# wangys16/FreeSplat

Measured on AMD Instinct MI355X. Metric: rendered views/sec @ 968x1296, 1.0M Gaussians, higher is better.
Workload: dtype f32

## Files before the change

### freesplat_amd/csrc/fs_common.h

```cpp
#pragma once
#include <hip/hip_runtime.h>
#include <stdint.h>

#include "../../include/freesplat_amd.h"

#define FS_API extern "C" __attribute__((visibility("default")))

namespace fs {

constexpr int kTile = FS_TILE;
constexpr int kTilePix = kTile * kTile;
constexpr int kWave = 64;

void set_last_error(const char* what, hipError_t e);

#define FS_CHECK_LAUNCH(what)                                   \
    do {                                                        \
        hipError_t e__ = hipGetLastError();                     \
        if (e__ != hipSuccess) {                                \
            fs::set_last_error(what, e__);                      \
            return FS_ERR_LAUNCH;                               \
        }                                                       \
    } while (0)

enum Stage {
    kStPreprocess = 0, kStTileScan, kStRender, kStRenderBwd, kStPreprocessBwd,
    kStCostVolume, kStPtf, kStEncoderTail, kNumStages
};
struct ScopedStage {
    ScopedStage(Stage s, hipStream_t st, int units = 1);
    ~ScopedStage();
    int slot_;
    hipStream_t st_;
};

__host__ __device__ inline size_t align_up(size_t x, size_t a) { return (x + a - 1) / a * a; }

constexpr float kExpC1 = 0.9999997019767761f, kExpC2 = 0.4999915063381195f, kExpC3 = 0.1666763573884964f, kExpC4 = 0.04189793020486832f, kExpC5 = 0.008290314115583897f;
__device__ __forceinline__ float fs_exp(float x)
{
    if (x < -80.0f) return 0.0f;
    const float t = fmaf(x, 1.44269504088896341f, 12582912.0f);
    const float n = t - 12582912.0f;
    const float r = fmaf(n, -0.693147182464599609375f, x);
    float p = fmaf(r, kExpC5, kExpC4);
    p = fmaf(r, p, kExpC3);
    p = fmaf(r, p, kExpC2);
    p = fmaf(r, p, kExpC1);
    p = fmaf(r, p, 1.0f);
    return ldexpf(p, (int)n);
}

#ifdef FS_PHASE_TRACE
constexpr int kPtKernels = 4, kPtBlocks = 4096, kPtSlots = 10;
static __device__ unsigned long long g_phase_trace[kPtKernels * kPtBlocks * kPtSlots];
#define FS_PT(kern, k)                                                                                  \
    do {                                                                                                \
        if (threadIdx.x == 0 && blockIdx.x < fs::kPtBlocks)                                             \
            fs::g_phase_trace[((kern) * fs::kPtBlocks + blockIdx.x) * fs::kPtSlots + (k)] = wall_clock64(); \
    } while (0)
#else
#define FS_PT(kern, k) do {} while (0)
#endif

__device__ __forceinline__ void rev2pi(float x, float& rev, float& res)
{
    constexpr float kInv2PiHi = 0.15915494f, kInv2PiLo = 6.4206382e-9f;
    rev = x * kInv2PiHi;
    res = fmaf(x, kInv2PiLo, fmaf(x, kInv2PiHi, -rev));
}
__device__ __forceinline__ void pos_enc2(float a, float b, float* __restrict__ out)
{
    float ra, ea, rb, eb;
    rev2pi(a, ra, ea);
    rev2pi(b, rb, eb);
#pragma unroll
    for (int k = 0; k < 6; ++k) {
        const float f = (float)(1 << k);
        const float ta = ra * f, tb = rb * f;
        const float pa = (ta - rintf(ta)) + ea * f, pb = (tb - rintf(tb)) + eb * f;
        out[2 * k] = __builtin_amdgcn_sinf(pa); out[2 * k + 1] = __builtin_amdgcn_cosf(pa);
        out[12 + 2 * k] = __builtin_amdgcn_sinf(pb); out[12 + 2 * k + 1] = __builtin_amdgcn_cosf(pb);
    }
}

int launch_ptf_gru(int n_max, const int32_t* counts, const float* cat, const float* tables, float* fused, hipStream_t st);
int launch_ptf_gru_gather(int n_max, const int32_t* counts, const long long* fuse_idx, const long long* fuse_pix,
                          const float* G, const float* R, const float* O, const float* g_i, const float* rho_i,
                          const float* om_i, const float* tables, float* fused, bool out_after_keep, hipStream_t st,
                          float* save_side = nullptr, float* save_act = nullptr, float* save_cat = nullptr);

__device__ __forceinline__ void wave_lds_sync()
{
    __builtin_amdgcn_fence(__ATOMIC_RELEASE, "wavefront");
    __builtin_amdgcn_wave_barrier();
    __builtin_amdgcn_fence(__ATOMIC_ACQUIRE, "wavefront");
}

typedef float f32x2 __attribute__((ext_vector_type(2)));
typedef int i32x2 __attribute__((ext_vector_type(2)));
__device__ __forceinline__ f32x2 fma2(f32x2 a, f32x2 b, f32x2 c) { return __builtin_elementwise_fma(a, b, c); }
__device__ __forceinline__ f32x2 splat2(float v) { return (f32x2){v, v}; }

__device__ __forceinline__ f32x2 fs_exp2_nonpos(f32x2 x)
{
    const f32x2 magic = splat2(12582912.0f);
    const f32x2 t = fma2(x, splat2(1.44269504088896341f), magic);
    const f32x2 n = t - magic;
    const f32x2 r = fma2(n, splat2(-0.693147182464599609375f), x);
    f32x2 q = fma2(r, splat2(kExpC5), splat2(kExpC4));
    q = fma2(r, q, splat2(kExpC3));
    q = fma2(r, q, splat2(kExpC2));
    q = fma2(r, q, splat2(kExpC1));
    q = fma2(r, q, splat2(1.0f));
    const i32x2 e = __builtin_bit_cast(i32x2, q) + (__builtin_bit_cast(i32x2, t) << 23);
    return __builtin_bit_cast(f32x2, e);
}

__device__ __forceinline__ f32x2 fs_exp2_of_neg(f32x2 q)
{
    const f32x2 magic = splat2(12582912.0f);
    const f32x2 t = fma2(q, splat2(-1.44269504088896341f), magic);
    const f32x2 n = t - magic;
    const f32x2 r = fma2(n, splat2(-0.693147182464599609375f), -q);
    f32x2 p = fma2(r, splat2(kExpC5), splat2(kExpC4));
    p = fma2(r, p, splat2(kExpC3));
    p = fma2(r, p, splat2(kExpC2));
    p = fma2(r, p, splat2(kExpC1));
    p = fma2(r, p, splat2(1.0f));
    const i32x2 e = __builtin_bit_cast(i32x2, p) + (__builtin_bit_cast(i32x2, t) << 23);
    return __builtin_bit_cast(f32x2, e);
}
template <bool FAST>
__device__ __forceinline__ f32x2 blend_exp_of_neg(f32x2 q)
{
    if constexpr (FAST) {
        const f32x2 t = q * splat2(-1.44269504088896341f);
// ... 223 lines not shown
```

### freesplat_amd/csrc/raster_fwd.hip

```cpp
#include <stdlib.h>

#include <type_traits>

#include "fs_common.h"

namespace fs {

template <int M>
__device__ __forceinline__ uint32_t lane_xor(uint32_t v)
{
    if constexpr (M == 1) return (uint32_t)__builtin_amdgcn_mov_dpp((int)v, 0xB1, 0xF, 0xF, true);
    else if constexpr (M == 2) return (uint32_t)__builtin_amdgcn_mov_dpp((int)v, 0x4E, 0xF, 0xF, true);
    else if constexpr (M == 3) return (uint32_t)__builtin_amdgcn_mov_dpp((int)v, 0x1B, 0xF, 0xF, true);
    else if constexpr (M < 32) return (uint32_t)__builtin_amdgcn_ds_swizzle((int)v, (M << 10) | 0x1F);
    else return (uint32_t)__shfl_xor((int)v, M, 64);
}
template <int M>
__device__ __forceinline__ unsigned long long lane_xor64(unsigned long long v)
{
    const uint32_t lo = lane_xor<M>((uint32_t)v), hi = lane_xor<M>((uint32_t)(v >> 32));
    return ((unsigned long long)hi << 32) | lo;
}

template <int DEG>
__device__ __forceinline__ void eval_sh(const float* __restrict__ sh, float3 dir, float* rgb,
                                        uint8_t& clampbits, int cs, int ks)
{
    float b[16];
    sh_basis<DEG>(dir.x, dir.y, dir.z, b);
    constexpr int NB = (DEG + 1) * (DEG + 1);
    clampbits = 0;
#pragma unroll
    for (int c = 0; c < 3; ++c) {
        const float* s = sh + c * cs;
        float acc = b[0] * s[0];
#pragma unroll
        for (int k = 1; k < NB; ++k) acc = acc + b[k] * s[k * ks];
        acc = acc + 0.5f;
        if (acc < 0.0f) clampbits |= (uint8_t)(1u << c);
        rgb[c] = fmaxf(acc, 0.0f);
    }
}

__device__ __forceinline__ void stage_rows(float* lds, const float* __restrict__ src, size_t base,
                                           int cnt, int per)
{
    const float* s = src + base * per;
    const int total = cnt * per;
    if ((((uintptr_t)s) & 15) == 0) {
        const int nv = total >> 2;
        int k = threadIdx.x;
        for (; k + 768 < nv; k += 1024) {
            const float4 v0 = ((const float4*)s)[k], v1 = ((const float4*)s)[k + 256];
            const float4 v2 = ((const float4*)s)[k + 512], v3 = ((const float4*)s)[k + 768];
            ((float4*)lds)[k] = v0; ((float4*)lds)[k + 256] = v1;
            ((float4*)lds)[k + 512] = v2; ((float4*)lds)[k + 768] = v3;
        }
        for (; k < nv; k += 256) ((float4*)lds)[k] = ((const float4*)s)[k];
        for (int k = (nv << 2) + threadIdx.x; k < total; k += blockDim.x) lds[k] = s[k];
    } else {
        for (int k = threadIdx.x; k < total; k += blockDim.x) lds[k] = s[k];
    }
}



struct QuadForm {
    float a, b, c;
    float Q;
    float D;
    float vplus;
    float Vmax;
    float inv2a;
};
__device__ __forceinline__ QuadForm quad_form(const float4 r0, const float4 r1)
{
    QuadForm f;
    f.a = -r0.z; f.c = -r0.w; f.b = -r1.x;
    f.Q = -(r1.z - 1e-3f * (1.0f + fabsf(r1.z)));
    f.D = 4.0f * f.a * f.c - f.b * f.b;
    const float invD = __builtin_amdgcn_rcpf(f.D);
    const float U = __builtin_amdgcn_sqrtf(fmaxf(4.0f * f.c * f.Q * invD, 0.0f));
    f.vplus = -f.b * __builtin_amdgcn_rcpf(2.0f * f.c) * U;
    f.Vmax = __builtin_amdgcn_sqrtf(fmaxf(4.0f * f.a * f.Q * invD, 0.0f));
    f.inv2a = __builtin_amdgcn_rcpf(2.0f * f.a);
    return f;
}
struct Band { float uL, uR; };
constexpr float kEps = 2e-5f;
__device__ __forceinline__ Band band_interval(const QuadForm& f, float vlo, float vhi)
{
    Band o;
    if (f.Q < 0.0f || vlo > f.Vmax + kEps || vhi < -f.Vmax - kEps) { o.uL = 3.0e38f; o.uR = -3.0e38f; return o; }
    const float vr = fminf(vhi, fmaxf(vlo, f.vplus)), vl = fminf(vhi, fmaxf(vlo, -f.vplus));
    const float sr = __builtin_amdgcn_sqrtf(fmaxf(4.0f * f.a * f.Q - f.D * vr * vr, 0.0f));
    const float sl = __builtin_amdgcn_sqrtf(fmaxf(4.0f * f.a * f.Q - f.D * vl * vl, 0.0f));
    o.uR = (-f.b * vr + sr) * f.inv2a;
    o.uL = (-f.b * vl - sl) * f.inv2a;
    const float w = kEps * (1.0f + fabsf(o.uR) + fabsf(o.uL));
    o.uR += w; o.uL -= w;
    return o;
}
struct RowBands { Band top, bot; };
__device__ __forceinline__ RowBands row_bands(const QuadForm& f, const float4 r0, int ty)
{
    const float v0 = (float)(ty * kTile) - r0.y;
    RowBands r;
    r.top = band_interval(f, v0, v0 + 7.0f);
    r.bot = band_interval(f, v0 + 8.0f, v0 + 15.0f);
    return r;
}
__device__ __forceinline__ uint32_t quad_mask_row(const RowBands& rb, const float4 r0, int tx)
{
    const float u0 = (float)(tx * kTile) - r0.x, u1 = u0 + 8.0f;
    uint32_t m = 0;
    if (!(u0 > rb.top.uR) && !(u0 + 7.0f < rb.top.uL)) m |= 1u;
    if (!(u1 > rb.top.uR) && !(u1 + 7.0f < rb.top.uL)) m |= 2u;
    if (!(u0 > rb.bot.uR) && !(u0 + 7.0f < rb.bot.uL)) m |= 4u;
    if (!(u1 > rb.bot.uR) && !(u1 + 7.0f < rb.bot.uL)) m |= 8u;
    return m;
}

__device__ __forceinline__ uint32_t band_cells(const Band& b, float px, int cell0, int ncell)
{
    const uint32_t full = ncell >= 32 ? 0xFFFFFFFFu : ((1u << ncell) - 1u);
    if (b.uL > b.uR) return 0u;
    if (!(b.uL <= b.uR)) return full;
    const float lo_f = ceilf((b.uL + px - 7.0f) * 0.125f - 1e-3f), hi_f = floorf((b.uR + px) * 0.125f + 1e-3f);
    const int lo = max((int)lo_f, cell0) - cell0, hi = min((int)hi_f, cell0 + ncell - 1) - cell0;
    if (lo > hi) return 0u;
    return ((2u << hi) - (1u << lo)) & full;
}
__device__ __forceinline__ unsigned long long pack_quad_masks(const QuadForm& f, const float4 r0, ushort4 rc)
{
    unsigned long long m = 0;
    const int rw = rc.z - rc.x, cell0 = 2 * rc.x, ncell = 2 * rw;
    int k = 0;
    for (int y = rc.y; y < rc.w; ++y) {
        const RowBands rb = row_bands(f, r0, y);
        const uint32_t top = band_cells(rb.top, r0.x, cell0, ncell), bot = band_cells(rb.bot, r0.x, cell0, ncell);
        for (int x = 0; x < rw; ++x, ++k) {
            const uint32_t nib = ((top >> (2 * x)) & 3u) | (((bot >> (2 * x)) & 3u) << 2);
            m |= (unsigned long long)nib << (4 * k);
        }
    }
    return m;
}

__device__ __forceinline__ uint32_t spread2(uint32_t x)
{
    x = (x | (x << 4)) & 0x0F0Fu;
    return (x | (x << 2)) & 0x3333u;
}
__device__ __forceinline__ unsigned long long pack_quad_masks4(const QuadForm& f, const float4 r0, ushort4 rc, bool cull, uint32_t& nz)
{
    unsigned long long m = 0;
    const int rw = rc.z - rc.x, rh = rc.w - rc.y, cell0 = 2 * rc.x, ncell = 2 * rw;
    const uint32_t rowfull = (1u << rw) - 1u;
    nz = 0u;
#pragma unroll
    for (int r = 0; r < 4; ++r) {
        if (r < rh) {
            const RowBands rb = row_bands(f, r0, rc.y + r);
            const uint32_t top = band_cells(rb.top, r0.x, cell0, ncell), bot = band_cells(rb.bot, r0.x, cell0, ncell);
            m |= (unsigned long long)(spread2(top) | (spread2(bot) << 2)) << (16 * r);
            uint32_t any = top | bot;
            any = (any | (any >> 1)) & 0x55u;
            any = (any | (any >> 1)) & 0x33u;
            any = (any | (any >> 2)) & 0x0Fu;
            nz |= (cull ? any : rowfull) << (4 * r);
        }
    }
    return m;
}

__device__ __forceinline__ void stage_rows_half(float* lds, const _Float16* __restrict__ src, size_t base, int cnt,
                                                int per)
{
    const _Float16* s = src + base * per;
    const int total = cnt * per;
    typedef _Float16 half8 __attribute__((ext_vector_type(8)));
    int done = 0;
    if ((((uintptr_t)s) & 15) == 0) {
        const int nv = total >> 3;
        auto put = [&](int k, const half8 v) {
            ((float4*)lds)[2 * k] = make_float4((float)v[0], (float)v[1], (float)v[2], (float)v[3]);
            ((float4*)lds)[2 * k + 1] = make_float4((float)v[4], (float)v[5], (float)v[6], (float)v[7]);
        };
        int k = threadIdx.x;
        for (; k + 256 < nv; k += 512) {
            const half8 v0 = ((const half8*)s)[k], v1 = ((const half8*)s)[k + 256];
            put(k, v0); put(k + 256, v1);
        }
        for (; k < nv; k += 256) put(k, ((const half8*)s)[k]);
        done = nv << 3;
    }
    for (int k = done + threadIdx.x; k < total; k += blockDim.x) lds[k] = (float)s[k];
}

struct Projected {
    float4 r0, r1, r2;
    ushort4 rect;
    uint8_t cb;
    int rad;
};
__device__ __forceinline__ Projected project_gaussian(
    const fs_raster_dims& d, bool live, float3 p_in, const float (&c_in)[6], float op, size_t i,
    const float* __restrict__ colors, const float* sh , int sh_cs, int sh_ks,
    const float* __restrict__ view, const float* __restrict__ proj, const float* __restrict__ campos,
    float tanfovx, float tanfovy, bool rescale, float wscale)
{
    Projected o;
    o.r0 = make_float4(0, 0, 0, 0); o.r1 = o.r0; o.r2 = o.r0;
    o.rect = make_ushort4(0, 0, 0, 0);
    o.cb = 0;
    o.rad = 0;
    float3 p = p_in;
    if (rescale) { p.x = p.x * wscale; p.y = p.y * wscale; p.z = p.z * wscale; }
    const float3 pv = xform43(view, p);
    if (live && pv.z > 0.2f) {
        const float4 ph = xform44(proj, p);
        const float pw = 1.0f / (ph.w + 0.0000001f);
        const float ndcx = ph.x * pw, ndcy = ph.y * pw;
        const float fx = (float)d.W / (2.0f * tanfovx), fy = (float)d.H / (2.0f * tanfovy);
        float c3[6];
#pragma unroll
        for (int k = 0; k < 6; ++k) c3[k] = c_in[k];
        if (rescale) {
            const float s2 = wscale * wscale;
#pragma unroll
            for (int k = 0; k < 6; ++k) c3[k] = c3[k] * s2;
        }
        const Cov2D cv = project_cov(view, p, c3, fx, fy, tanfovx, tanfovy);
        const float det = cv.a * cv.c - cv.b * cv.b;
        if (det != 0.0f) {
            const float det_inv = 1.0f / det;
            const float cA = cv.c * det_inv, cB = -cv.b * det_inv, cC = cv.a * det_inv;
            const float mid = 0.5f * (cv.a + cv.c);
            const float sq = sqrtf(fmaxf(0.1f, mid * mid - det));
            const float l1 = mid + sq, l2 = mid - sq;
            const float my_radius = ceilf(3.0f * sqrtf(fmaxf(l1, l2)));
            const float px = ((ndcx + 1.0f) * (float)d.W - 1.0f) * 0.5f;
            const float py = ((ndcy + 1.0f) * (float)d.H - 1.0f) * 0.5f;
            const int r = (int)my_radius;
            const int gx = (d.W + kTile - 1) / kTile, gy = (d.H + kTile - 1) / kTile;
            const int x0 = min(gx, max(0, (int)((px - (float)r) / (float)kTile)));
            const int y0 = min(gy, max(0, (int)((py - (float)r) / (float)kTile)));
            const int x1 = min(gx, max(0, (int)((px + (float)r + (float)(kTile - 1)) / (float)kTile)));
            const int y1 = min(gy, max(0, (int)((py + (float)r + (float)(kTile - 1)) / (float)kTile)));
            if ((x1 - x0) * (y1 - y0) > 0) {
                float rgb[3];
                if (colors) {
                    rgb[0] = colors[3 * i];
                    rgb[1] = colors[3 * i + 1];
                    rgb[2] = colors[3 * i + 2];
                } else {
                    float3 dir = make_float3(p.x - campos[0], p.y - campos[1], p.z - campos[2]);
                    const float len = sqrtf(dir.x * dir.x + dir.y * dir.y + dir.z * dir.z);
                    dir.x = dir.x / len; dir.y = dir.y / len; dir.z = dir.z / len;
                    switch (d.sh_degree) {
                        case 0: eval_sh<0>(sh, dir, rgb, o.cb, sh_cs, sh_ks); break;
                        case 1: eval_sh<1>(sh, dir, rgb, o.cb, sh_cs, sh_ks); break;
                        case 2: eval_sh<2>(sh, dir, rgb, o.cb, sh_cs, sh_ks); break;
                        default: eval_sh<3>(sh, dir, rgb, o.cb, sh_cs, sh_ks); break;
                    }
                }
                float thr;
                if (op > 0.0f) {
                    const float l = -logf(255.0f * op);
                    thr = l - (0.001f + 1e-5f * fabsf(l));
                } else {
                    thr = 1.0f;
                }
                o.r0 = make_float4(px, py, -0.5f * cA, -0.5f * cC);
                o.r1 = make_float4(-cB, op, thr, pv.z);
                o.r2 = make_float4(rgb[0], rgb[1], rgb[2], 0.0f);
                o.rect = make_ushort4((unsigned short)x0, (unsigned short)y0, (unsigned short)x1,
                                      (unsigned short)y1);
                o.rad = r;
            }
        }
    }
    return o;
}

template <bool SR>
__device__ __forceinline__ void load_mean_cov(const fs_raster_dims& d, const float* __restrict__ means3D,
                                              const float* __restrict__ cov3D, size_t i, float3& p_in, float (&c_in)[6])
{
    p_in = make_float3(means3D[3 * i], means3D[3 * i + 1], means3D[3 * i + 2]);
    if constexpr (SR) {
        float row[7];
#pragma unroll
        for (int k = 0; k < 7; ++k) row[k] = cov3D[7 * i + k];
        cov_from_scale_rot(row, c_in);
    } else if (d.flags & FS_RASTER_COV_FULL) {
        const float* cr = cov3D + 9 * i;
        c_in[0] = cr[0]; c_in[1] = cr[1]; c_in[2] = cr[2]; c_in[3] = cr[4]; c_in[4] = cr[5]; c_in[5] = cr[8];
    } else {
#pragma unroll
        for (int k = 0; k < 6; ++k) c_in[k] = cov3D[6 * i + k];
    }
}

constexpr int kWaveBins = 512;

__device__ __forceinline__ void bin_wave(const fs_raster_dims& d, int lane, uint32_t* s_cnt, uint32_t i, const Projected& pr,
                                         uint32_t* __restrict__ tile_counts, unsigned long long* __restrict__ keys,
                                         uint32_t tile_cap)
{
    const float4 r0 = pr.r0, r1 = pr.r1;
    const ushort4 rect = pr.rect;
    const bool valid = pr.rad > 0;
    const bool cull = (d.flags & FS_RASTER_TILE_CULL) != 0;
    const int gx = (d.W + kTile - 1) / kTile;
    const QuadForm qf = quad_form(r0, r1);
    const int rw = rect.z - rect.x, rh = rect.w - rect.y;
    const int area = rw * rh;
    const bool small = area <= 16;
    const bool all4 = __builtin_amdgcn_ballot_w64(valid && (rw > 4 || rh > 4)) == 0ull;
    unsigned long long qm = 0;
    uint32_t nz = 0u;
    if (all4) { if (valid) qm = pack_quad_masks4(qf, r0, rect, cull, nz); }
    else if (valid && small) qm = pack_quad_masks(qf, r0, rect);
    const unsigned long long key_hi = ((unsigned long long)__float_as_uint(r1.w) << 32) | (i << 4);
    int x0 = valid ? (int)rect.x : 0x7fff, y0 = valid ? (int)rect.y : 0x7fff;
    int x1 = valid ? (int)rect.z : 0, y1 = valid ? (int)rect.w : 0;
#define FS_BOX_STEP(M)                                                                                           \
    {                                                                                                            \
        const int lo = (int)lane_xor<M>((uint32_t)((x0 << 16) | y0)), hi = (int)lane_xor<M>((uint32_t)((x1 << 16) | y1)); \
        x0 = min(x0, lo >> 16); y0 = min(y0, lo & 0xffff);                                                       \
        x1 = max(x1, hi >> 16); y1 = max(y1, hi & 0xffff);                                                       \
    }
    FS_BOX_STEP(32) FS_BOX_STEP(16) FS_BOX_STEP(8) FS_BOX_STEP(4) FS_BOX_STEP(2) FS_BOX_STEP(1)
#undef FS_BOX_STEP
    const int bx0 = __builtin_amdgcn_readfirstlane(x0), by0 = __builtin_amdgcn_readfirstlane(y0);
    const int bw = max(0, __builtin_amdgcn_readfirstlane(x1) - bx0), bh = max(0, __builtin_amdgcn_readfirstlane(y1) - by0);
    const int nb = bw * bh;
    if (nb == 0) return;
    if (nb <= kWaveBins && all4) {
        for (int k = lane; k < nb; k += 64) s_cnt[k] = 0u;
        wave_lds_sync();
        const int cbase = (rect.y - by0) * bw + (rect.x - bx0);
        for (uint32_t z = nz; z != 0u; z &= z - 1u) {
            const int k = __builtin_ctz(z);
            atomicAdd(&s_cnt[cbase + (k >> 2) * bw + (k & 3)], 1u);
        }
        wave_lds_sync();
        for (int k0 = 0; k0 < nb; k0 += 64) {
            const int k = k0 + lane;
            if (k < nb) {
                const uint32_t c = s_cnt[k];
                const int ky = k / bw, kx = k - ky * bw;
                s_cnt[k] = c ? atomicAdd(&tile_counts[(by0 + ky) * gx + bx0 + kx], c) : 0u;
            }
        }
        wave_lds_sync();
        const uint32_t tbase = (uint32_t)(rect.y * gx + rect.x);
        for (uint32_t z = nz; z != 0u; z &= z - 1u) {
            const int k = __builtin_ctz(z);
            const uint32_t m = (uint32_t)(qm >> (4 * k)) & 15u;
            const uint32_t slot = atomicAdd(&s_cnt[cbase + (k >> 2) * bw + (k & 3)], 1u);
            if (slot < tile_cap) keys[(tbase + (uint32_t)((k >> 2) * gx + (k & 3))) * tile_cap + slot] = key_hi | m;
        }
        wave_lds_sync();
    } else if (nb <= kWaveBins) {
        for (int k = lane; k < nb; k += 64) s_cnt[k] = 0u;
        wave_lds_sync();
        if (valid) {
            int k = 0;
            for (int y = rect.y; y < rect.w; ++y) {
                RowBands rb = {};
                if (!small) rb = row_bands(qf, r0, y);
                for (int x = rect.x; x < rect.z; ++x, ++k) {
                    const uint32_t m = small ? (uint32_t)(qm >> (4 * k)) & 15u : quad_mask_row(rb, r0, x);
                    if (!cull || m) atomicAdd(&s_cnt[(y - by0) * bw + (x - bx0)], 1u);
                }
            }
        }
        wave_lds_sync();
        for (int k0 = 0; k0 < nb; k0 += 64) {
            const int k = k0 + lane;
            if (k < nb) {
                const uint32_t c = s_cnt[k];
                const int ky = k / bw, kx = k - ky * bw;
                s_cnt[k] = c ? atomicAdd(&tile_counts[(by0 + ky) * gx + bx0 + kx], c) : 0u;
            }
        }
        wave_lds_sync();
        if (valid) {
            int k = 0;
            for (int y = rect.y; y < rect.w; ++y) {
                RowBands rb = {};
                if (!small) rb = row_bands(qf, r0, y);
                for (int x = rect.x; x < rect.z; ++x, ++k) {
                    const uint32_t m = small ? (uint32_t)(qm >> (4 * k)) & 15u : quad_mask_row(rb, r0, x);
                    if (!cull || m) {
                        const uint32_t slot = atomicAdd(&s_cnt[(y - by0) * bw + (x - bx0)], 1u);
                        if (slot < tile_cap) keys[(uint32_t)(y * gx + x) * tile_cap + slot] = key_hi | m;
                    }
                }
            }
        }
        wave_lds_sync();
    } else if (all4) {
        const uint32_t tbase = (uint32_t)(rect.y * gx + rect.x);
        for (uint32_t z = nz; z != 0u; z &= z - 1u) {
            const int k = __builtin_ctz(z);
            const uint32_t m = (uint32_t)(qm >> (4 * k)) & 15u;
            const uint32_t tile = tbase + (uint32_t)((k >> 2) * gx + (k & 3));
            const uint32_t slot = atomicAdd(&tile_counts[tile], 1u);
            if (slot < tile_cap) keys[tile * tile_cap + slot] = key_hi | m;
        }
    } else if (valid) {
        int k = 0;
        for (int y = rect.y; y < rect.w; ++y) {
            RowBands rb = {};
            if (!small) rb = row_bands(qf, r0, y);
            for (int x = rect.x; x < rect.z; ++x, ++k) {
                const uint32_t m = small ? (uint32_t)(qm >> (4 * k)) & 15u : quad_mask_row(rb, r0, x);
                if (!cull || m) {
                    const uint32_t slot = atomicAdd(&tile_counts[y * gx + x], 1u);
                    if (slot < tile_cap) keys[(uint32_t)(y * gx + x) * tile_cap + slot] = key_hi | m;
                }
            }
        }
    }
}

__global__ __launch_bounds__(256) void zero_counts_kernel(char* base, size_t stride, int T)
{
    const int k = blockIdx.x * 256 + threadIdx.x;
    if (k < T) ((uint32_t*)(base + stride * blockIdx.y))[k] = 0u;
}

struct ViewBuffers {
    char* geom; size_t geom_stride;
    char* scratch; size_t scratch_stride;
    int32_t* radii;
};

#ifndef FS_PRE_WAVES
#define FS_PRE_WAVES 6
#endif
#define FS_PRE_OCC __attribute__((amdgpu_waves_per_eu(FS_PRE_WAVES, FS_PRE_WAVES)))
template <int CH, bool SR>
__global__ __launch_bounds__(256) FS_PRE_OCC void preprocess_views_kernel(
    fs_raster_dims d, int v, const float* __restrict__ means3D, const float* __restrict__ cov3D,
    const float* __restrict__ shs, const float* __restrict__ colors, const float* __restrict__ opacities,
    const float* __restrict__ view, const float* __restrict__ proj, const float* __restrict__ campos,
    const float* __restrict__ tanfov_dev, const float* __restrict__ scale_dev, ViewBuffers vb, uint32_t tile_cap)
{
    extern __shared__ __attribute__((aligned(16))) float lds[];
    constexpr int kPerBlock = 64 * CH;
    const int base = blockIdx.x * kPerBlock;
    const int cnt = min(kPerBlock, d.N - base);
    const int per_sh = shs ? d.M * 3 : 0;
    const bool sh_cm = (d.flags & FS_RASTER_SH_CHANNEL_MAJOR) != 0;
    const int sh_cs = sh_cm ? d.M : 1, sh_ks = sh_cm ? 1 : 3;
    float* const l_sh = lds;
    if (shs) {
        if (d.flags & FS_RASTER_SH_FP16) stage_rows_half(l_sh, (const _Float16*)shs, base, cnt, per_sh);
        else stage_rows(l_sh, shs, base, cnt, per_sh);
    }
    const int t = threadIdx.x, lane = t & 63, wave = t >> 6;
    const int chunk = wave % CH;
    uint32_t* const s_cnt_base = (uint32_t*)(lds + (size_t)kPerBlock * per_sh);
    uint32_t* const s_cnt = s_cnt_base + wave * kWaveBins;
    const int li = chunk * 64 + lane;
    const bool live = li < cnt;
    const uint32_t i = (uint32_t)(base + li);
    float* const l_g = (float*)(s_cnt_base + 4 * kWaveBins) + li;
    {
        float3 p_in = make_float3(0.0f, 0.0f, 0.0f);
        float c_in[6] = {0, 0, 0, 0, 0, 0};
        float op = 0.0f;
        if (live) {
            load_mean_cov<SR>(d, means3D, cov3D, i, p_in, c_in);
            op = opacities[i];
        }
        if (wave < CH) {
            l_g[0 * kPerBlock] = p_in.x; l_g[1 * kPerBlock] = p_in.y; l_g[2 * kPerBlock] = p_in.z;
#pragma unroll
            for (int k = 0; k < 6; ++k) l_g[(3 + k) * kPerBlock] = c_in[k];
            l_g[9 * kPerBlock] = op;
        }
    }
    __syncthreads();
    const int T = num_tiles(d.H, d.W);
    const size_t keys_off = align_up((size_t)T * 4, 256);
#pragma nounroll
    for (int j0 = wave / CH; j0 < v; j0 += 4 / CH) {
        const int j = __builtin_amdgcn_readfirstlane(j0);
        int li_ = li, lane_ = lane;
        asm volatile("" : "+v"(li_), "+v"(lane_));
        const float* const lg = (const float*)(s_cnt_base + 4 * kWaveBins) + li_;
        const float3 p_in = make_float3(lg[0 * kPerBlock], lg[1 * kPerBlock], lg[2 * kPerBlock]);
        float c_in[6];
#pragma unroll
        for (int k = 0; k < 6; ++k) c_in[k] = lg[(3 + k) * kPerBlock];
        const float op = lg[9 * kPerBlock];
        const float tanfovx = tanfov_dev ? tanfov_dev[2 * j] : d.tanfovx;
        const float tanfovy = tanfov_dev ? tanfov_dev[2 * j + 1] : d.tanfovy;
        const float wscale = scale_dev ? scale_dev[j] : 1.0f;
        const Projected pr = project_gaussian(d, live, p_in, c_in, op, i, colors, l_sh + (size_t)li_ * per_sh, sh_cs, sh_ks,
                                              view + 16 * j, proj + 16 * j, campos + 3 * j, tanfovx, tanfovy,
                                              scale_dev != nullptr, wscale);
        if (live) {
            const GeomView g = geom_view(vb.geom + vb.geom_stride * j, d.N);
            g.rec[3 * (size_t)i + 0] = pr.r0;
            g.rec[3 * (size_t)i + 1] = pr.r1;
            g.rec[3 * (size_t)i + 2] = pr.r2;
            if (!(d.flags & FS_RASTER_NO_BACKWARD_STATE)) {
                g.rect[i] = pr.rect;
                g.clamp[i] = pr.cb;
            }
            if (vb.radii) vb.radii[(size_t)j * d.N + i] = pr.rad;
        }
        char* const sc = vb.scratch + vb.scratch_stride * j;
        bin_wave(d, lane_, s_cnt, i, pr, (uint32_t*)sc, (unsigned long long*)(sc + keys_off), tile_cap);
    }
}

__global__ __launch_bounds__(1024) void tile_scan_kernel(const char* __restrict__ counts0, size_t counts_stride,
                                                         char* __restrict__ offsets0, size_t offsets_stride, int T,
                                                         uint32_t* __restrict__ counters0,
                                                         unsigned long long cap, uint32_t tile_cap)
{
    const uint32_t* __restrict__ counts = (const uint32_t*)(counts0 + counts_stride * blockIdx.x);
    uint32_t* __restrict__ offsets = (uint32_t*)(offsets0 + offsets_stride * blockIdx.x);
    uint32_t* __restrict__ counters = counters0 + 2 * blockIdx.x;
    __shared__ uint32_t s_wave[16];
    __shared__ uint32_t s_max[16];
    __shared__ unsigned long long s_wide[16];
    const int t = threadIdx.x, lane = t & 63, wave = t >> 6;
    const int per = (T + 1023) / 1024;
    const int lo = min(T, t * per), hi = min(T, lo + per);
    uint32_t s = 0, mx = 0;
    unsigned long long wide = 0;
    for (int k = lo; k < hi; ++k) { const uint32_t c = counts[k]; s += c; wide += c; mx = max(mx, c); }
#pragma unroll
    for (int d = 32; d >= 1; d >>= 1) {
        wide += __shfl_xor(wide, d, 64);
        mx = max(mx, (uint32_t)__shfl_xor((int)mx, d, 64));
    }
    if (lane == 0) { s_wide[wave] = wide; s_max[wave] = mx; }
    uint32_t inc = s;
#pragma unroll
    for (int d = 1; d < 64; d <<= 1) {
        const uint32_t o = __shfl_up(inc, d, 64);
        if (lane >= d) inc += o;
    }
    if (lane == 63) s_wave[wave] = inc;
    __syncthreads();
    uint32_t before = 0, total = 0;
#pragma unroll
    for (int k = 0; k < 16; ++k) {
        const uint32_t v = s_wave[k];
        before += k < wave ? v : 0u;
        total += v;
    }
    inc += before;
    uint32_t run = inc - s;
    for (int k = lo; k < hi; ++k) {
        offsets[k] = run;
        run += counts[k];
    }
    if (t == 1023) {
        unsigned long long total64 = 0;
        uint32_t maxc = 0;
#pragma unroll
        for (int k = 0; k < 16; ++k) { total64 += s_wide[k]; maxc = max(maxc, s_max[k]); }
        offsets[T] = total;
        counters[0] = total64 > 0xFFFFFFFFull ? 0xFFFFFFFFu : (uint32_t)total64;
        counters[1] = (total64 > cap || maxc > tile_cap) ? max(maxc, 1u) : 0u;
    }
}

#ifndef FS_SORT_LDS
#define FS_SORT_LDS 1792
#endif
constexpr int kSortLds = FS_SORT_LDS;

template <typename Ptr>
__device__ __forceinline__ void bitonic_sort_any(Ptr a, uint32_t n)
{
    uint32_t P = 1;
    while (P < n) P <<= 1;
    const uint32_t half = P >> 1;
    for (uint32_t k = 2; k <= P; k <<= 1) {
        const uint32_t hk = k >> 1;
        for (uint32_t t = threadIdx.x; t < half; t += blockDim.x) {
            const uint32_t blk = t / hk, off = t % hk;
            const uint32_t i = blk * k + off, j = blk * k + (k - 1 - off);
            if (j < n) {
                const unsigned long long x = a[i], y = a[j];
                if (x > y) { a[i] = y; a[j] = x; }
            }
        }
        __syncthreads();
        for (uint32_t s = k >> 2; s >= 1; s >>= 1) {
// ... 491 lines not shown
        blend_quadrant<FAST_EXP, TRACK, false>(gl, (int)n, rec, cp, H, W, tx, ty, wave, bg, out_color, out_depth, out_alpha,
                                               final_T, n_contrib);
    FS_PT(2, 3);
}

}

using namespace fs;

FS_API int fs_raster_buffer_sizes(int32_t N, int32_t H, int32_t W, int64_t cap, size_t out[4])
{
    if (N < 0 || H <= 0 || W <= 0 || cap < 0 || !out) return FS_ERR_INVALID_ARG;
    const size_t T = (size_t)num_tiles(H, W), P = (size_t)H * W;
    out[0] = geom_bytes(N > 0 ? N : 1);
    out[1] = binning_offsets_bytes(H, W) + align_up((size_t)(cap > 0 ? cap : 1) * 4, 256);
    out[2] = align_up(P * 4, 256) * 2;
    out[3] = align_up(T * 4, 256) + align_up(T * (size_t)tile_capacity(cap, (int)T) * 8, 256);
    return FS_OK;
}

FS_API const uint32_t* fs_raster_tile_ranges(const void* binning, int32_t, int32_t)
{
    return (const uint32_t*)binning;
}
FS_API const uint32_t* fs_raster_point_list(const void* binning, int32_t H, int32_t W)
{
    return (const uint32_t*)((const char*)binning + binning_offsets_bytes(H, W));
}
FS_API const float* fs_raster_geom_records(const void* geom) { return (const float*)geom; }
FS_API const float* fs_raster_final_T(const void* image) { return (const float*)image; }
FS_API const int32_t* fs_raster_n_contrib(const void* image, int32_t H, int32_t W)
{
    return (const int32_t*)((const char*)image + align_up((size_t)H * W * 4, 256));
}

namespace fs {
constexpr int kMaxViewsInFlight = 16;
static int raster_batch()
{
    static const int n = [] {
        const char* e = getenv("FREESPLAT_RASTER_BATCH");
        const int x = e ? atoi(e) : 16;
        return x < 1 ? 1 : (x > kMaxViewsInFlight ? kMaxViewsInFlight : x);
    }();
    return n;
}

static int check_forward_args(const fs_raster_dims& d, const float* means3D, const float* cov3D, const float* shs,
                              const float* colors_precomp, const float* opacities, const int32_t* radii, int64_t cap)
{
    if (d.N < 0 || d.H <= 0 || d.W <= 0 || cap < 1) return FS_ERR_INVALID_ARG;
    if ((d.flags & FS_RASTER_SCALE_ROT) && (d.flags & FS_RASTER_COV_FULL)) return FS_ERR_INVALID_ARG;
    if (d.N > 0) {
        if (!means3D || !cov3D || !opacities || !radii) return FS_ERR_INVALID_ARG;
        if ((shs == nullptr) == (colors_precomp == nullptr)) return FS_ERR_INVALID_ARG;
    }
    if (shs && (d.sh_degree < 0 || d.sh_degree > 3 || (d.sh_degree + 1) * (d.sh_degree + 1) > d.M))
        return FS_ERR_UNSUPPORTED;
    const int gx = (d.W + kTile - 1) / kTile, gy = (d.H + kTile - 1) / kTile;
    if (gx > 32767 || gy > 32767) return FS_ERR_UNSUPPORTED;
    if (d.N > (1 << 28)) return FS_ERR_UNSUPPORTED;
    if (cap > 0xFFFFFFFFll) return FS_ERR_UNSUPPORTED;
    return FS_OK;
}

static int launch_binning(const fs_raster_dims& d, int nv, const float* means3D, const float* cov3D, const float* shs,
                          const float* colors_precomp, const float* opacities, const float* viewmatrix,
                          const float* projmatrix, const float* campos, const float* tanfov, const float* scale,
                          void* geom, size_t geom_stride, void* binning, size_t binning_stride, void* scratch,
                          size_t scratch_stride, int64_t cap, int32_t* radii, uint32_t* counters, hipStream_t st)
{
    const int T = num_tiles(d.H, d.W);
    const uint32_t tile_cap = tile_capacity(cap, T);
    hipLaunchKernelGGL(zero_counts_kernel, dim3((T + 255) / 256, nv), dim3(256), 0, st, (char*)scratch, scratch_stride, T);
    FS_CHECK_LAUNCH("zero tile counts");
    if (d.N > 0) {
        const int M = shs ? d.M : 0;
        ViewBuffers vb;
        vb.geom = (char*)geom; vb.geom_stride = geom_stride;
        vb.scratch = (char*)scratch; vb.scratch_stride = scratch_stride;
        vb.radii = radii;
        const int ch = nv >= 4 ? 1 : (nv == 2 ? 2 : 4);
        const size_t lds = (size_t)(64 * ch * M * 3) * sizeof(float) + (size_t)4 * kWaveBins * sizeof(uint32_t)
                           + (size_t)(10 * 64 * ch) * sizeof(float);
        const dim3 grid((d.N + 64 * ch - 1) / (64 * ch));
        ScopedStage prof_(kStPreprocess, st, nv);
#define FS_LAUNCH_PRE(CH, SR)                                                                                        \
        hipLaunchKernelGGL((preprocess_views_kernel<CH, SR>), grid, dim3(256), lds, st, d, nv, means3D, cov3D, shs,  \
                           colors_precomp, opacities, viewmatrix, projmatrix, campos, tanfov, scale, vb, tile_cap)
        if (d.flags & FS_RASTER_SCALE_ROT) {
            if (ch == 1) FS_LAUNCH_PRE(1, true); else if (ch == 2) FS_LAUNCH_PRE(2, true); else FS_LAUNCH_PRE(4, true);
        } else {
            if (ch == 1) FS_LAUNCH_PRE(1, false); else if (ch == 2) FS_LAUNCH_PRE(2, false); else FS_LAUNCH_PRE(4, false);
        }
#undef FS_LAUNCH_PRE
    }
    FS_CHECK_LAUNCH("preprocess_views");
    {
        ScopedStage prof_(kStTileScan, st, nv);
        hipLaunchKernelGGL(tile_scan_kernel, dim3(nv), dim3(1024), 0, st, (const char*)scratch, scratch_stride,
                           (char*)binning, binning_stride, T, counters, (unsigned long long)cap, tile_cap);
    }
    FS_CHECK_LAUNCH("tile_scan");
    return FS_OK;
}

static int launch_blend(const fs_raster_dims& d, const float* bg, void* geom, void* binning, void* image, void* scratch,
                        int64_t cap, float* out_color, float* out_depth, float* out_alpha, const uint32_t* counters,
                        hipStream_t st)
{
    const int gx = (d.W + kTile - 1) / kTile, gy = (d.H + kTile - 1) / kTile;
    const int T = gx * gy;
    const size_t P = (size_t)d.H * d.W;
    const GeomView g = geom_view(geom, d.N > 0 ? d.N : 1);
    uint32_t* offsets = (uint32_t*)binning;
    uint32_t* point_list = (uint32_t*)((char*)binning + binning_offsets_bytes(d.H, d.W));
    float* final_T = (float*)image;
    int32_t* n_contrib = (int32_t*)((char*)image + align_up(P * 4, 256));
    uint32_t* counts = (uint32_t*)scratch;
    unsigned long long* keys = (unsigned long long*)((char*)scratch + align_up((size_t)T * 4, 256));
    const uint32_t tile_cap = tile_capacity(cap, T);
    const int nblk = tile_grid_blocks(gx, gy);
    {
        ScopedStage prof_(kStRender, st);
#define FS_LAUNCH_RENDER(F, TR)                                                                                     \
        hipLaunchKernelGGL((sort_blend_kernel<F, TR>), dim3(nblk), dim3(256), 0, st, d.H, d.W, counts, offsets, tile_cap, \
                           keys, point_list, g.rec, bg, counters, out_color, out_depth, out_alpha, final_T, n_contrib)
        const bool track = !(d.flags & FS_RASTER_NO_BACKWARD_STATE);
        if (d.flags & FS_RASTER_FAST_EXP) { if (track) FS_LAUNCH_RENDER(true, true); else FS_LAUNCH_RENDER(true, false); }
        else { if (track) FS_LAUNCH_RENDER(false, true); else FS_LAUNCH_RENDER(false, false); }
#undef FS_LAUNCH_RENDER
    }
    FS_CHECK_LAUNCH("sort_blend");
    return FS_OK;
}

__global__ __launch_bounds__(256) void cov3d_from_scale_rot_kernel(int N, const float* __restrict__ rows,
                                                                   float* __restrict__ cov)
{
    for (int i = blockIdx.x * 256 + threadIdx.x; i < N; i += gridDim.x * 256) {
        float row[7], c[6];
#pragma unroll
        for (int k = 0; k < 7; ++k) row[k] = rows[7 * (size_t)i + k];
        cov_from_scale_rot(row, c);
#pragma unroll
        for (int k = 0; k < 6; ++k) cov[6 * (size_t)i + k] = c[k];
    }
}
}

FS_API int fs_raster_cov3d_from_scale_rot(int32_t N, const float* rows7, float* cov6_out, void* stream_)
{
    if (N < 0) return FS_ERR_INVALID_ARG;
    if (N == 0) return FS_OK;
    if (!rows7 || !cov6_out) return FS_ERR_INVALID_ARG;
    const int nb = (N + 255) / 256;
    const unsigned blocks = (unsigned)(nb < 8192 ? nb : 8192);
    hipLaunchKernelGGL(fs::cov3d_from_scale_rot_kernel, dim3(blocks), dim3(256), 0, (hipStream_t)stream_, N, rows7, cov6_out);
    FS_CHECK_LAUNCH("cov3d_from_scale_rot");
    return FS_OK;
}

FS_API int fs_raster_forward(const fs_raster_dims* dims, const float* means3D, const float* cov3D,
                             const float* shs, const float* colors_precomp, const float* opacities,
                             const float* bg, const float* viewmatrix, const float* projmatrix,
                             const float* campos, const float* tanfov_dev, const float* scale_dev,
                             void* geom, void* binning, void* image, void* scratch, int64_t cap, float* out_color, float* out_depth,
// ... 111 lines not shown
```

### profiles/phase_trace.py

```python
#!/usr/bin/env python
import ctypes as C
import os
import sys

import numpy as np
import torch

ROOT = os.path.dirname(os.path.dirname(os.path.abspath(__file__)))
sys.path.insert(0, ROOT)
from freesplat_amd import _lib, synthetic
from freesplat_amd.decoder import render_views

PHASES = {
    0: ("preprocess (projection + binning)", ["stage inputs + sync", "project / conic / SH", "write records + sync", "quadrant masks",
                       "workgroup box", "zero + count (LDS atomics)", "reserve slots (returning global atomics)",
                       "rank + write keys"]),
    2: ("sort_blend (wavefront 0)", ["load keys + LDS bucket sort", "wait for the other wavefronts", "blend quadrant 0"]),
}


def main():
    dev = torch.device("cuda:0")
    H, W, N = synthetic.WORKLOADS["c3_968x1296_1M"]
    scene = synthetic.make_scene(N)
    cams = {k: v[:1].to(dev) for k, v in synthetic.target_cameras(8).items()}
    g = {k: scene[k].to(dev) for k in ("means", "covariances", "harmonics", "opacities")}
    L = _lib.lib()
    L.fs_debug_phase_trace.restype = C.c_int
    buf = np.zeros(4 * 4096 * 10, np.uint64)
    with torch.no_grad():
        for it in range(4):
            render_views(cams["extrinsics"], cams["intrinsics"], cams["near"], cams["far"], (H, W), torch.zeros(1, 3, device=dev),
                         g["means"], g["covariances"], g["harmonics"], g["opacities"])
            torch.cuda.synchronize()
            L.fs_debug_phase_trace(buf.ctypes.data_as(C.c_void_p))
    t = buf.reshape(4, 4096, 10).astype(np.float64) / 100.0
    for kern, (name, phases) in PHASES.items():
        n = len(phases) + 1
        x = t[kern][:, :n]
        x = x[(x > 0).all(axis=1)]
        if not len(x):
            print(f"{name}: no samples")
            continue
        d = np.diff(x, axis=1)
        print(f"{name}: {len(x)} workgroups, {(x[:, -1] - x[:, 0]).mean():.2f} us each")
        for ph, m, md in zip(phases, d.mean(0), np.median(d, 0)):
            print(f"   {ph:34s} mean {m:6.2f} us   median {md:6.2f}")


if __name__ == "__main__":
    main()
```

Measured before the change: 4460.

## Streamline preprocess binning: hoisted band constants, packed box reduce, per-Gaussian threshold

Several micro-optimisations land in the preprocess/binning kernel. The quadrant-mask builder now computes the per-Gaussian band constants once and uses a branchless band_cells4 per row. The wavefront bounding-box reduction uses packed u16 min/max on combined words instead of four separate shuffles and mins. The opacity skip threshold (a logf) is computed once per Gaussian during staging rather than per view. A float reciprocal also replaces the integer divide when mapping bins to tiles. These trade extra LDS (one more float slot per Gaussian) and possible floating-point edge cases in the reciprocal indexing for fewer ALU ops. Phase-trace instrumentation points are added as well.

```diff
diff --git a/freesplat_amd/csrc/fs_common.h b/freesplat_amd/csrc/fs_common.h
--- a/freesplat_amd/csrc/fs_common.h
+++ b/freesplat_amd/csrc/fs_common.h
@@ -52,7 +52,7 @@
 }
 
 #ifdef FS_PHASE_TRACE
-constexpr int kPtKernels = 4, kPtBlocks = 4096, kPtSlots = 10;
+constexpr int kPtKernels = 4, kPtBlocks = 4096, kPtSlots = 12;
 static __device__ unsigned long long g_phase_trace[kPtKernels * kPtBlocks * kPtSlots];
 #define FS_PT(kern, k)                                                                                  \
     do {                                                                                                \
diff --git a/freesplat_amd/csrc/raster_fwd.hip b/freesplat_amd/csrc/raster_fwd.hip
--- a/freesplat_amd/csrc/raster_fwd.hip
+++ b/freesplat_amd/csrc/raster_fwd.hip
@@ -20,6 +20,16 @@
 {
     const uint32_t lo = lane_xor<M>((uint32_t)v), hi = lane_xor<M>((uint32_t)(v >> 32));
     return ((unsigned long long)hi << 32) | lo;
+}
+
+typedef unsigned short ushort2_v __attribute__((ext_vector_type(2)));
+__device__ __forceinline__ uint32_t pk_min_u16(uint32_t a, uint32_t b)
+{
+    return __builtin_bit_cast(uint32_t, __builtin_elementwise_min(__builtin_bit_cast(ushort2_v, a), __builtin_bit_cast(ushort2_v, b)));
+}
+__device__ __forceinline__ uint32_t pk_max_u16(uint32_t a, uint32_t b)
+{
+    return __builtin_bit_cast(uint32_t, __builtin_elementwise_max(__builtin_bit_cast(ushort2_v, a), __builtin_bit_cast(ushort2_v, b)));
 }
 
 template <int DEG>
@@ -152,17 +162,40 @@
     x = (x | (x << 4)) & 0x0F0Fu;
     return (x | (x << 2)) & 0x3333u;
 }
+struct BandConsts { float a4Q, vtop, vbot, c0f, c1f; uint32_t full; bool dead; };
+__device__ __forceinline__ uint32_t band_cells4(const QuadForm& f, const BandConsts& k, float px, float vlo, float vhi)
+{
+    const bool empty = k.dead || vlo > k.vtop || vhi < k.vbot;
+    const float vr = fminf(vhi, fmaxf(vlo, f.vplus)), vl = fminf(vhi, fmaxf(vlo, -f.vplus));
+    const float sr = __builtin_amdgcn_sqrtf(fmaxf(k.a4Q - f.D * vr * vr, 0.0f));
+    const float sl = __builtin_amdgcn_sqrtf(fmaxf(k.a4Q - f.D * vl * vl, 0.0f));
+    float uR = (-f.b * vr + sr) * f.inv2a, uL = (-f.b * vl - sl) * f.inv2a;
+    const float w = kEps * (1.0f + fabsf(uR) + fabsf(uL));
+    uR += w; uL -= w;
+    const float lo_f = ceilf((uL + px - 7.0f) * 0.125f - 1e-3f), hi_f = floorf((uR + px) * 0.125f + 1e-3f);
+    const int lo = (int)(fmaxf(lo_f, k.c0f) - k.c0f), hi = (int)(fminf(hi_f, k.c1f) - k.c0f);
+    uint32_t m = ((2u << (hi & 31)) - (1u << (lo & 31))) & k.full;
+    m = lo > hi ? 0u : m;
+    m = uL <= uR ? m : (uL > uR ? 0u : k.full);
+    return empty ? 0u : m;
+}
 __device__ __forceinline__ unsigned long long pack_quad_masks4(const QuadForm& f, const float4 r0, ushort4 rc, bool cull, uint32_t& nz)
 {
     unsigned long long m = 0;
     const int rw = rc.z - rc.x, rh = rc.w - rc.y, cell0 = 2 * rc.x, ncell = 2 * rw;
     const uint32_t rowfull = (1u << rw) - 1u;
+    BandConsts k;
+    k.a4Q = 4.0f * f.a * f.Q;
+    k.vtop = f.Vmax + kEps; k.vbot = -f.Vmax - kEps;
+    k.c0f = (float)cell0; k.c1f = (float)(cell0 + ncell - 1);
+    k.full = (1u << ncell) - 1u;
+    k.dead = f.Q < 0.0f;
     nz = 0u;
 #pragma unroll
     for (int r = 0; r < 4; ++r) {
         if (r < rh) {
-            const RowBands rb = row_bands(f, r0, rc.y + r);
-            const uint32_t top = band_cells(rb.top, r0.x, cell0, ncell), bot = band_cells(rb.bot, r0.x, cell0, ncell);
+            const float v0 = (float)((rc.y + r) * kTile) - r0.y;
+            const uint32_t top = band_cells4(f, k, r0.x, v0, v0 + 7.0f), bot = band_cells4(f, k, r0.x, v0 + 8.0f, v0 + 15.0f);
             m |= (unsigned long long)(spread2(top) | (spread2(bot) << 2)) << (16 * r);
             uint32_t any = top | bot;
             any = (any | (any >> 1)) & 0x55u;
@@ -198,6 +231,15 @@
     for (int k = done + threadIdx.x; k < total; k += blockDim.x) lds[k] = (float)s[k];
 }
 
+__device__ __forceinline__ float skip_threshold(float op)
+{
+    if (op > 0.0f) {
+        const float l = -logf(255.0f * op);
+        return l - (0.001f + 1e-5f * fabsf(l));
+    }
+    return 1.0f;
+}
+
 struct Projected {
     float4 r0, r1, r2;
     ushort4 rect;
@@ -205,7 +247,7 @@
     int rad;
 };
 __device__ __forceinline__ Projected project_gaussian(
-    const fs_raster_dims& d, bool live, float3 p_in, const float (&c_in)[6], float op, size_t i,
+    const fs_raster_dims& d, bool live, float3 p_in, const float (&c_in)[6], float op, float thr, size_t i,
     const float* __restrict__ colors, const float* sh , int sh_cs, int sh_ks,
     const float* __restrict__ view, const float* __restrict__ proj, const float* __restrict__ campos,
     float tanfovx, float tanfovy, bool rescale, float wscale)
@@ -249,6 +291,7 @@
             const int x1 = min(gx, max(0, (int)((px + (float)r + (float)(kTile - 1)) / (float)kTile)));
             const int y1 = min(gy, max(0, (int)((py + (float)r + (float)(kTile - 1)) / (float)kTile)));
             if ((x1 - x0) * (y1 - y0) > 0) {
+                FS_PT(0, 2);
                 float rgb[3];
                 if (colors) {
                     rgb[0] = colors[3 * i];
@@ -265,13 +308,8 @@
                         default: eval_sh<3>(sh, dir, rgb, o.cb, sh_cs, sh_ks); break;
                     }
                 }
-                float thr;
-                if (op > 0.0f) {
-                    const float l = -logf(255.0f * op);
-                    thr = l - (0.001f + 1e-5f * fabsf(l));
-                } else {
-                    thr = 1.0f;
-                }
+                FS_PT(0, 3);
+                FS_PT(0, 4);
                 o.r0 = make_float4(px, py, -0.5f * cA, -0.5f * cC);
                 o.r1 = make_float4(-cB, op, thr, pv.z);
                 o.r2 = make_float4(rgb[0], rgb[1], rgb[2], 0.0f);
@@ -323,22 +361,20 @@
     uint32_t nz = 0u;
     if (all4) { if (valid) qm = pack_quad_masks4(qf, r0, rect, cull, nz); }
     else if (valid && small) qm = pack_quad_masks(qf, r0, rect);
+    FS_PT(0, 6);
     const unsigned long long key_hi = ((unsigned long long)__float_as_uint(r1.w) << 32) | (i << 4);
-    int x0 = valid ? (int)rect.x : 0x7fff, y0 = valid ? (int)rect.y : 0x7fff;
-    int x1 = valid ? (int)rect.z : 0, y1 = valid ? (int)rect.w : 0;
-#define FS_BOX_STEP(M)                                                                                           \
-    {                                                                                                            \
-        const int lo = (int)lane_xor<M>((uint32_t)((x0 << 16) | y0)), hi = (int)lane_xor<M>((uint32_t)((x1 << 16) | y1)); \
-        x0 = min(x0, lo >> 16); y0 = min(y0, lo & 0xffff);                                                       \
-        x1 = max(x1, hi >> 16); y1 = max(y1, hi & 0xffff);                                                       \
-    }
+    uint32_t lo = valid ? ((uint32_t)rect.x << 16) | rect.y : 0x7fff7fffu, hi = valid ? ((uint32_t)rect.z << 16) | rect.w : 0u;
+#define FS_BOX_STEP(M) { lo = pk_min_u16(lo, lane_xor<M>(lo)); hi = pk_max_u16(hi, lane_xor<M>(hi)); }
     FS_BOX_STEP(32) FS_BOX_STEP(16) FS_BOX_STEP(8) FS_BOX_STEP(4) FS_BOX_STEP(2) FS_BOX_STEP(1)
 #undef FS_BOX_STEP
-    const int bx0 = __builtin_amdgcn_readfirstlane(x0), by0 = __builtin_amdgcn_readfirstlane(y0);
-    const int bw = max(0, __builtin_amdgcn_readfirstlane(x1) - bx0), bh = max(0, __builtin_amdgcn_readfirstlane(y1) - by0);
+    lo = (uint32_t)__builtin_amdgcn_readfirstlane((int)lo); hi = (uint32_t)__builtin_amdgcn_readfirstlane((int)hi);
+    const int bx0 = (int)(lo >> 16), by0 = (int)(lo & 0xffffu);
+    const int bw = max(0, (int)(hi >> 16) - bx0), bh = max(0, (int)(hi & 0xffffu) - by0);
     const int nb = bw * bh;
+    FS_PT(0, 7);
     if (nb == 0) return;
     if (nb <= kWaveBins && all4) {
+        const float inv_bw = __builtin_amdgcn_rcpf((float)bw);
         for (int k = lane; k < nb; k += 64) s_cnt[k] = 0u;
         wave_lds_sync();
         const int cbase = (rect.y - by0) * bw + (rect.x - bx0);
@@ -347,15 +383,17 @@
             atomicAdd(&s_cnt[cbase + (k >> 2) * bw + (k & 3)], 1u);
         }
         wave_lds_sync();
+        FS_PT(0, 8);
         for (int k0 = 0; k0 < nb; k0 += 64) {
             const int k = k0 + lane;
             if (k < nb) {
                 const uint32_t c = s_cnt[k];
-                const int ky = k / bw, kx = k - ky * bw;
+                const int ky = (int)(((float)k + 0.5f) * inv_bw), kx = k - ky * bw;
                 s_cnt[k] = c ? atomicAdd(&tile_counts[(by0 + ky) * gx + bx0 + kx], c) : 0u;
             }
         }
         wave_lds_sync();
+        FS_PT(0, 9);
         const uint32_t tbase = (uint32_t)(rect.y * gx + rect.x);
         for (uint32_t z = nz; z != 0u; z &= z - 1u) {
             const int k = __builtin_ctz(z);
@@ -364,6 +402,7 @@
             if (slot < tile_cap) keys[(tbase + (uint32_t)((k >> 2) * gx + (k & 3))) * tile_cap + slot] = key_hi | m;
         }
         wave_lds_sync();
+        FS_PT(0, 10);
     } else if (nb <= kWaveBins) {
         for (int k = lane; k < nb; k += 64) s_cnt[k] = 0u;
         wave_lds_sync();
@@ -452,6 +491,7 @@
     const float* __restrict__ tanfov_dev, const float* __restrict__ scale_dev, ViewBuffers vb, uint32_t tile_cap)
 {
     extern __shared__ __attribute__((aligned(16))) float lds[];
+    FS_PT(0, 0);
     constexpr int kPerBlock = 64 * CH;
     const int base = blockIdx.x * kPerBlock;
     const int cnt = min(kPerBlock, d.N - base);
@@ -484,9 +524,11 @@
 #pragma unroll
             for (int k = 0; k < 6; ++k) l_g[(3 + k) * kPerBlock] = c_in[k];
             l_g[9 * kPerBlock] = op;
+            l_g[10 * kPerBlock] = skip_threshold(op);
         }
     }
     __syncthreads();
+    FS_PT(0, 1);
     const int T = num_tiles(d.H, d.W);
     const size_t keys_off = align_up((size_t)T * 4, 256);
 #pragma nounroll
@@ -499,11 +541,11 @@
         float c_in[6];
 #pragma unroll
         for (int k = 0; k < 6; ++k) c_in[k] = lg[(3 + k) * kPerBlock];
-        const float op = lg[9 * kPerBlock];
+        const float op = lg[9 * kPerBlock], thr = lg[10 * kPerBlock];
         const float tanfovx = tanfov_dev ? tanfov_dev[2 * j] : d.tanfovx;
         const float tanfovy = tanfov_dev ? tanfov_dev[2 * j + 1] : d.tanfovy;
         const float wscale = scale_dev ? scale_dev[j] : 1.0f;
-        const Projected pr = project_gaussian(d, live, p_in, c_in, op, i, colors, l_sh + (size_t)li_ * per_sh, sh_cs, sh_ks,
+        const Projected pr = project_gaussian(d, live, p_in, c_in, op, thr, i, colors, l_sh + (size_t)li_ * per_sh, sh_cs, sh_ks,
                                               view + 16 * j, proj + 16 * j, campos + 3 * j, tanfovx, tanfovy,
                                               scale_dev != nullptr, wscale);
         if (live) {
@@ -517,6 +559,7 @@
             }
             if (vb.radii) vb.radii[(size_t)j * d.N + i] = pr.rad;
         }
+        FS_PT(0, 5);
         char* const sc = vb.scratch + vb.scratch_stride * j;
         bin_wave(d, lane_, s_cnt, i, pr, (uint32_t*)sc, (unsigned long long*)(sc + keys_off), tile_cap);
     }
@@ -1174,7 +1217,7 @@
         vb.radii = radii;
         const int ch = nv >= 4 ? 1 : (nv == 2 ? 2 : 4);
         const size_t lds = (size_t)(64 * ch * M * 3) * sizeof(float) + (size_t)4 * kWaveBins * sizeof(uint32_t)
-                           + (size_t)(10 * 64 * ch) * sizeof(float);
+                           + (size_t)(11 * 64 * ch) * sizeof(float);
         const dim3 grid((d.N + 64 * ch - 1) / (64 * ch));
         ScopedStage prof_(kStPreprocess, st, nv);
 #define FS_LAUNCH_PRE(CH, SR)                                                                                        \
diff --git a/profiles/phase_trace.py b/profiles/phase_trace.py
--- a/profiles/phase_trace.py
+++ b/profiles/phase_trace.py
@@ -12,9 +12,10 @@
 from freesplat_amd.decoder import render_views
 
 PHASES = {
-    0: ("preprocess (projection + binning)", ["stage inputs + sync", "project / conic / SH", "write records + sync", "quadrant masks",
-                       "workgroup box", "zero + count (LDS atomics)", "reserve slots (returning global atomics)",
-                       "rank + write keys"]),
+    0: ("preprocess_views (projection + binning, wavefront 0)",
+        ["load and park + sync", "projection (conic, radius, rect)", "SH -> RGB", "skip threshold", "record stores",
+         "quadrant masks", "wavefront box", "zero + count (LDS atomics)", "reserve slots (returning global atomics)",
+         "key pass"]),
     2: ("sort_blend (wavefront 0)", ["load keys + LDS bucket sort", "wait for the other wavefronts", "blend quadrant 0"]),
 }
 
@@ -27,14 +28,14 @@
     g = {k: scene[k].to(dev) for k in ("means", "covariances", "harmonics", "opacities")}
     L = _lib.lib()
     L.fs_debug_phase_trace.restype = C.c_int
-    buf = np.zeros(4 * 4096 * 10, np.uint64)
+    buf = np.zeros(4 * 4096 * 12, np.uint64)
     with torch.no_grad():
         for it in range(4):
             render_views(cams["extrinsics"], cams["intrinsics"], cams["near"], cams["far"], (H, W), torch.zeros(1, 3, device=dev),
                          g["means"], g["covariances"], g["harmonics"], g["opacities"])
             torch.cuda.synchronize()
             L.fs_debug_phase_trace(buf.ctypes.data_as(C.c_void_p))
-    t = buf.reshape(4, 4096, 10).astype(np.float64) / 100.0
+    t = buf.reshape(4, 4096, 12).astype(np.float64) / 100.0
     for kern, (name, phases) in PHASES.items():
         n = len(phases) + 1
         x = t[kern][:, :n]
```

Result: no change. 4457 (median of 2 runs) (-0.1%).
